# osudrl/cassie-mujoco-sim

Hardware: AMD Instinct MI355X
Metric: env-steps/sec (whole node) at N envs; max |qpos_err| vs CPU ref (higher is better)
Workload: dtype f64

## Files before the change

### cassie-mujoco-sim_amd/csrc/env_step_wave1.inc

```
    if constexpr (NW == 2) {
        if (wid == 1) {
            for (int sub1 = sub_start;;) {
                const int pb = isbody ? b : 0;
                const double mass = P->body_mass[pb];
                double iner[3], imat[9];
                for (int i = 0; i < 3; ++i) iner[i] = P->body_inertia[pb][i];
                for (int i = 0; i < 9; ++i) imat[i] = m->body_imat[pb][i];
                CK_STAMP(35);
                wv::block_barrier();
                if (wv::opaque(S.cmd[0])) return -1;
                wv::set_priority<(FEAT & FEAT_HFIELD) != 0 ? CK_PRIO_W1_FJ_HFIELD : CK_PRIO_W1_FJ>();
                CK_STAMP(36);
                double ximat[9] = {1, 0, 0, 0, 1, 0, 0, 0, 1};
                if (isbody && b > 0) {
                    double xm[9];
                    for (int i = 0; i < 9; ++i) xm[i] = S.x.s.xmat[b][i];
                    for (int i = 0; i < 3; ++i)
                        for (int c = 0; c < 3; ++c) ximat[3 * i + c] = xm[3 * i] * imat[c] + xm[3 * i + 1] * imat[3 + c] + xm[3 * i + 2] * imat[6 + c];
                }
                double col[NVP], colh[NVP];
                mass_matrix_columns<NVP, TOPO, FEAT, NW>(io, S, m, env, ids, mass, iner, ximat, col, colh);
                wv::publish(&S.cmd[3], sub1 + 1);
                CK_STAMP(38);
                factor_pair_by_height<NVP, TOPO, 0>(m, P, h, S, col, colh, lane);
                constexpr bool park_colh = NVP > 32;
                if constexpr (park_colh) {
                    if (isdof) {
#pragma unroll
                        for (int i = 0; i < NVP; ++i) {
                            if (i >= TOPO::nv) continue;
                            if (i == k_) S.dinvH[k_] = colh[i];
                            else if (i > k_ && LP::col_has(i, k_)) S.LHp[LP::col_idx(i, k_)] = colh[i];
                        }
                    }
                    wv::sync();
                }
                wv::wait_for(&S.cmd[4], sub1 + 1);
                if (wv::opaque(S.cmd[0])) return -1;
                if (io.drive_mode) {
                    if (io.integrate) drive_level_io(io, S, m, env, lane, sub1 == nsub - 1);
                    wv::sync();
                }
                CK_STAMP(4);
                {
                    const int kd = isdof ? k_ : 0;
                    const double kdamp = P->dof_damping[kd], kstiff = PS->dof_stiffness[kd], kref = PS->dof_springref[kd];
                    const double kgear = m->dof_gear[kd], klo = m->dof_ctrl_lo[kd], khi = m->dof_ctrl_hi[kd];
                    const int kq = m->dof_qadr[kd], ka = m->dof_act[kd];
                    wv::wait_for(&S.cmd[1], sub1 + 1);
                    bias_forces_and_qfrc_smooth<NVP, (NVP > 32)>(io, S, m, env, ids, kdamp, kstiff, kref, kgear, klo, khi, kq, ka);
                }
                const bool lastsub1 = sub1 == nsub - 1 || !io.integrate;
                const bool need_imu1 = lastsub1 || io.all_outputs_every_substep || (io.drive_mode && sub1 + 2 == nsub);
                const bool issens1 = lane < m->nsensor && (lastsub1 || io.drive_mode || io.all_outputs_every_substep);
                const int ls1 = issens1 ? lane : 0;
                const SensorConsts sens_c1 = request_sensor_consts(m, ls1);
                const int aslot1 = sensors_before_solve(io, S, m, env, issens1, ls1, sens_c1, need_imu1, lastsub1);
                CK_STAMP(47);
                wv::block_barrier();
                wv::set_priority<CK_PRIO_W1_JP>();
                CK_STAMP(39);
                if constexpr (WIDE) {
                    int it1 = 0, ng1 = 0;
                    const double f1 = wide_solve<NVP, TOPO>(S, m, P, 1, wv::opaque(S.x.turn[0]), sub1, it1, ng1);
                    (&S.c_solimp[0][0])[NROW + lane] = f1;
                }
                if constexpr (park_colh) {
#pragma unroll
                    for (int i = 0; i < NVP; ++i) {
                        double v = 0.0;
                        if (i < TOPO::nv && isdof) {
                            if (i == k_) v = S.dinvH[k_];
                            else if (i > k_ && LP::col_has(i, k_)) v = S.LHp[LP::col_idx(i, k_)];
                        }
                        colh[i] = v;
                    }
                    wv::sync();
                }
                factor_pair_by_height<NVP, TOPO, 1>(m, P, h, S, col, colh, lane);
                {
                    const bool lastsub = lastsub1, need_imu = need_imu1;
                    const int sb = sens_c1.sb, aslot = aslot1;
                    const int pf_u = lane < nu ? lane : 0, pf_ej = lane < njnt ? lane : 0;
                    const double pf_agear = m->act_gear[pf_u], pf_kdamp = P->dof_damping[isdof ? k_ : 0];
                    const int pf_adof = m->act_dofid[pf_u], pf_ejt = m->jnt_type[pf_ej], pf_eqa = m->jnt_qposadr[pf_ej], pf_eda = m->jnt_dofadr[pf_ej];
                    const double *const fbuf = &S.c_solimp[0][0];
                    double lrow[NVP];
                    constexpr bool stage_h_early = NVP <= 32;
                    if constexpr (stage_h_early) stage_factor_row<NVP, TOPO>(S, k_, isdof, lrow);
                    double lcol[NVP], lrowh[NVP];
                    if constexpr (stage_h_early) stage_factor_h<NVP, TOPO, 0>(S, k_, isdof, nv, lcol, lrowh);
                    const double rsdk = isdof ? S.rsd[k_] : 0.0;
                    const int kk = isdof ? k_ : 0;
                    constexpr bool stage_y = MAXR <= 31;
                    double ycolk[stage_y ? MAXR + 1 : 1];
                    if constexpr (stage_y) {
                        wv::wait_for(&S.cmd[2], sub1 + 1);
#pragma unroll
                        for (int r = 0; r <= MAXR; ++r) ycolk[r] = S.x.Yr[r][kk];
                    }
                    wv::block_barrier();
                    wv::set_priority<CK_PRIO_W1_PE>();
                    const double f = fbuf[lane], f_hi = WIDE ? fbuf[NROW + lane] : 0.0;
                    constexpr int FB = WIDE ? 2 * NROW : NROW;
                    const int ncon = (int)fbuf[FB], nefc = (int)fbuf[FB + 1], iters = (int)fbuf[FB + 2], nguarded = (int)fbuf[FB + 3];
                    double z, z1 = 0, z2 = 0, z3 = 0;
                    if constexpr (stage_y) {
                        z = isdof ? ycolk[MAXR] : 0.0;
#pragma unroll
                        for (int r = 0; r < MAXR; r += 4) {
                            if (r + 4 <= nefc) {
                                z += ycolk[r] * wv::readlane(f, r); z1 += ycolk[r + 1 < MAXR ? r + 1 : r] * wv::readlane(f, r + 1);
                                z2 += ycolk[r + 2 < MAXR ? r + 2 : r] * wv::readlane(f, r + 2); z3 += ycolk[r + 3 < MAXR ? r + 3 : r] * wv::readlane(f, r + 3);
                            } else {
#pragma unroll
                                for (int j = 0; j < 4; ++j) if (r + j < nefc && r + j < MAXR) z += ycolk[r + j < MAXR ? r + j : r] * wv::readlane(f, r + j);
                            }
                        }
                    } else {
                        z = isdof ? S.x.Yr[MAXR][k_] : 0.0;
                        auto frow = [&](int r) { if constexpr (WIDE) return r < NROW ? wv::readlane(f, r) : wv::readlane(f_hi, r - NROW); else return wv::readlane(f, r); };
                        int r = 0;
                        for (; r + 4 <= nefc; r += 4) {
                            const double y0 = S.x.Yr[r][kk], y1 = S.x.Yr[r + 1][kk], y2 = S.x.Yr[r + 2][kk], y3 = S.x.Yr[r + 3][kk];
                            z += y0 * frow(r); z1 += y1 * frow(r + 1);
                            z2 += y2 * frow(r + 2); z3 += y3 * frow(r + 3);
                        }
                        for (; r < nefc; ++r) z += S.x.Yr[r][kk] * frow(r);
                    }
                    z = (z + z1) + (z2 + z3);
                    if (!isdof) z = 0.0;
                    if (isdof) z *= rsdk;
                    if constexpr (stage_h_early) stage_factor_h<NVP, TOPO, 1>(S, k_, isdof, nv, lcol, lrowh);
                    const double dih = isdof ? S.dinvH[k_] : 0.0;
                    if constexpr (!stage_h_early) stage_factor_row<NVP, TOPO>(S, k_, isdof, lrow);
                    wv::sched_fence();
                    const double qacc = solve_forward<NVP, TOPO>(z, lrow, lane, nv);
                    {
                        const bool badv = isdof && (!(qacc == qacc) || fabs(qacc) > 1e10);
                        if (wv::ballot(badv) != 0ull) {
                            if (lane == 0) S.cmd[0] = 2;
                            wv::block_barrier();
                            return -1;
                        }
                    }
                    if (isdof) S.qacc[k_] = qacc;
                    const double av = pf_agear * S.qvel[pf_adof];
                    wv::sync();
                    CK_STAMP(12);
                    if (io.integrate) {
                        if constexpr (!stage_h_early) stage_factor_h<NVP, TOPO>(S, k_, isdof, nv, lcol, lrowh);
                        euler_step<NVP, TOPO>(S, m, lane, isdof, k_, nv, njnt, h, qacc, lcol, lrowh, dih, pf_kdamp, pf_ejt, pf_eqa, pf_eda);
                    }
                    CK_STAMP(13);
                    wv::block_barrier();
                    wv::set_priority<CK_PRIO_W1_EF>();
                    outputs_after_qacc(io, S, m, env, lane, isdof, k_, nu, qacc, aslot, sb, need_imu, lastsub, av, ncon, nefc, iters, nguarded);
                    CK_STAMP(14);
                }
                if (!io.integrate || ++sub1 >= nsub) return -1;
            }
        }
    }
```

### cassie-mujoco-sim_amd/csrc/physics_kernel.h

```cpp
#ifndef CASSIE_PHYSICS_KERNEL_H
#define CASSIE_PHYSICS_KERNEL_H

#include <wave.h>

#include "cm_model.h"
#include "topo_static.h"

#include "pk_types.h"
#include "pk_math.h"
#include "pk_safety.h"
#include "pk_collision.h"
#include "pk_factor_solve.h"
#include "pk_stages.h"
#include "pk_wide_solve.h"

namespace ck {


constexpr int ENV_STEP_WENT_DOWN = 1 << 20;

template <int NVP, class TOPO, int FEAT, int MAXR, int NW>
WV_DEVICE int env_step(const PhysIO &io, EnvShared<NVP, LPack<TOPO, NVP>::count, MAXR> &S, int env, int sub_start, int nsub) {
    typedef LPack<TOPO, NVP> LP;
    static_assert(NW == 1 || NW == 2, "one or two wavefronts per env");
    static_assert(NW == 1 || TOPO::is_static, "the two-wave form exists for the compile-time topologies");
    const int wid = NW == 2 ? wv::wave_id() : 0;
    if constexpr (NW == 2) { if (wid == 0) wv::set_priority<CK_PRIO_W0>(); }
    constexpr int prio_kin = (FEAT & FEAT_HFIELD) != 0 ? CK_PRIO_W0 : CK_PRIO_W0_KIN;

    static_assert(LP::covers() && LP::distinct(), "packed factor rows must hold every ancestor pair, each in its own slot");
    typedef EnvShared<NVP, LPack<TOPO, NVP>::count, MAXR> SH_T;
    constexpr int MAXC = SH_T::MAXC;
    constexpr bool WIDE = SH_T::WIDE;
    static_assert(!WIDE || (NW == 2 && MAXR == WIDE_ROWS), "the 127-row instantiation spreads its solve over the two wavefronts of an env");
    const ModelPtr m_launch = (ModelPtr)(io.models + (size_t)env * io.model_stride);
    ModelPtr m = m_launch;
    const ParamPtr P = io.envparams ? (ParamPtr)(io.envparams + (size_t)env) : (ParamPtr)&m_launch->params;
    const ParamPtr PG = m_launch->env_geom ? P : (ParamPtr)&m_launch->params, PS = m_launch->env_springs ? P : (ParamPtr)&m_launch->params;
    int lane = wv::lane();
    const int nq = m->nq, nv = m->nv, nu = m->nu, nbody = m->nbody, njnt = m->njnt;
    const int capr = m->maxefc < MAXR ? m->maxefc : MAXR, capc = m->maxcon < MAXC ? m->maxcon : MAXC;
    const bool can_hand_over = MAXR < WIDE_ROWS && io.has_next != 0 && io.progress != nullptr && (MAXR < m->maxefc || MAXC < m->maxcon);
    const double h = m->timestep;
    int warn = 0;

    if (NW == 1 || wid == 0) {
    if (lane == 0) { S.cmd[0] = 0; S.cmd[1] = 0; S.cmd[2] = 0; S.cmd[3] = 0; S.cmd[4] = 0; }
    if constexpr (WIDE) { if (lane == 0) { S.x.turn[0] = 0; S.x.turn[1] = 0; S.x.turn[2] = 0; S.x.turn[3] = 0; } }
    if (lane < nq) S.qpos[lane] = io.qpos[(size_t)env * io.sq + lane];
    if (lane < nv) {
        S.qvel[lane] = io.qvel[(size_t)env * io.sqv + lane];
        S.qacc_ws[lane] = io.qacc_warmstart[(size_t)env * io.sv + lane];
    }
    if (lane < nu) S.ctrl[lane] = io.ctrl[(size_t)env * io.su + lane];
    if (lane < NB && !wv::test_skip_com_init()) { S.com[lane][0] = 0.0; S.com[lane][1] = 0.0; S.com[lane][2] = 0.0; }
    if (io.drive_mode) {
        if (lane < m->nsensordata) S.sens[lane] = io.sensordata[(size_t)env * io.ssd + lane];
        if (lane < nu) S.actvel[lane] = io.actuator_velocity[(size_t)env * io.su + lane];
        drive_state_load(io, S, env, lane);
        drive_consts_load(io, S, m, env, lane);
    }
    }
    double time = io.time[env];

    int b = lane;
    bool isbody = b < nbody;
    const int depth = isbody ? m->body_depth[b] : -1;
    const int bparent = isbody ? m->body_parentid[b] : 0;
    const int broot = isbody ? m->body_rootid[b] : -1;
    const int bjn = isbody ? m->body_jntnum[b] : 0;
    const int bj0 = (isbody && bjn > 0) ? m->body_jntadr[b] : 0;
    const int bend = isbody ? m->body_subtreeend[b] : 0;
    const unsigned long long bdofmask = isbody ? m->body_dofmask[b] : 0ull;
    const int bjt = (isbody && bjn > 0) ? m->jnt_type[bj0] : -1;
    const int bjq = (isbody && bjn > 0) ? m->jnt_qposadr[bj0] : 0;
    int k_ = lane;
    bool isdof = k_ < nv;
    const int kjnt = isdof ? m->dof_jntid[k_] : 0;
    const int kbody = isdof ? m->dof_bodyid[k_] : 0;
    const int kjt = isdof ? m->jnt_type[kjnt] : -1;
    const int kda = isdof ? m->jnt_dofadr[kjnt] : 0;
    const int kqa = isdof ? m->jnt_qposadr[kjnt] : 0;
    const int kroot = isdof ? m->body_rootid[kbody] : 0;
    const int kbend = isdof ? m->body_subtreeend[kbody] : 0;
    const unsigned long long kdesc = isdof ? m->dof_descmask[k_] : 0ull;
    const unsigned long long kvelmask = isdof ? m->dof_velmask[k_] : 0ull;
    int kact = -1;
    for (int u = 0; u < nu; ++u) if (isdof && m->act_dofid[u] == k_) kact = u;
    const LaneIds ids = {nbody, nv, broot, bend, kjnt, kbody, kjt, kda, kroot, kbend, kdesc};
    wv::sync();

#include "env_step_wave1.inc"

    const float *env_hfield = nullptr;
    if constexpr ((FEAT & FEAT_HFIELD) != 0) {
        bool clamped;
        env_hfield = terrain_grid(io.hfield, io.hfield_stride, io.hfield_index, io.hfield_nterrain, env, &clamped);
        if (clamped && lane == 0 && wid == 0) wv::atomic_or(io.warn + env, WARN_TERRAIN_INDEX);
    }

    bool bailed = false, bailed_down = false;
    int sub = sub_start;
    for (; sub < nsub; ++sub) {
        const bool lastsub = sub == nsub - 1 || !io.integrate;
        const bool need_quat = lastsub || io.ext != nullptr || io.all_outputs_every_substep || (io.drive_mode && sub + 2 == nsub);
        {
            bool badv = false;
            if (lane < nq) { double v = S.qpos[lane]; badv |= !(v == v) || fabs(v) > 1e10; }
            if (lane < nv) { double v = S.qvel[lane]; badv |= !(v == v) || fabs(v) > 1e10; }
            if (wv::ballot(badv) != 0ull) {
                warn |= WARN_DIVERGED;
                if constexpr (NW == 2) { if (lane == 0) S.cmd[0] = 1; wv::block_barrier(); }
                break;
            }
        }
        if (io.drive_mode) {
        } else if (io.pd_ptarget) {
            if (lane < nu) {
                const size_t o = (size_t)env * io.su + lane;
                const double ratio = m->act_gear[lane], tmax = m->act_ctrlrange[lane][1];
                const double q = S.qpos[m->act_qposadr[lane]], qd = S.qvel[m->act_dofid[lane]];
                const double tau = io.pd_kp[o] * (io.pd_ptarget[o] - q) - io.pd_kd[o] * qd;
                const double wmax = m->act_maxrpm[lane] * (2.0 * 3.14159265358979323846 / 60.0);
                const double tlim = clampd(2 * tmax * (1 - fabs(ratio * qd) / wmax), 0.0, tmax);
                S.ctrl[lane] = copysign(fmin(fabs(tau / ratio), tlim), tau);
            }
            wv::sync();
        }
        CK_STAMP(0);
        if constexpr (NW == 2 && prio_kin != CK_PRIO_W0) wv::set_priority<prio_kin>();

        double Rl[9] = {1, 0, 0, 0, 1, 0, 0, 0, 1}, pl[3] = {0, 0, 0}, qlq[4] = {1, 0, 0, 0};
        constexpr int kin_rounds = [] {
            if constexpr (TOPO::is_static) { int r = 0, n = 1; while (n < TOPO::body_levels) { n *= 3; ++r; } return r < 1 ? 1 : r; }
            else return 3;
        }();
        int kanc[2 * kin_rounds];
#pragma unroll
        for (int r = 0; r < 2 * kin_rounds; ++r) kanc[r] = isbody ? m->body_anc3[b][r] : 0;
        const bool isfree = bjt == CM_JNT_FREE;
        if constexpr (TOPO::is_static) {
            {
                const auto *kr = &m->body_kin[isbody ? b : 0];
                const int nsl = kr->nslide, j0 = kr->jnt0, jr = kr->rot_jnt, jt = kr->rot_type, qa = kr->rot_qadr;
                int sqa[CM_MAXSLIDE];
                double sref[CM_MAXSLIDE], sax[CM_MAXSLIDE][3], spo[CM_MAXSLIDE][3];
#pragma unroll
                for (int sl = 0; sl < CM_MAXSLIDE; ++sl) {
                    sqa[sl] = kr->slide_qadr[sl]; sref[sl] = kr->slide_ref[sl];
                    for (int i = 0; i < 3; ++i) { sax[sl][i] = kr->slide_axis_p[sl][i]; spo[sl][i] = kr->slide_pos_p[sl][i]; }
                }
                const double jref = kr->rot_ref;
                double jp[3], ja[3], jpp[3], xl[3], q0[4];
                for (int i = 0; i < 3; ++i) { jp[i] = kr->rot_pos[i]; ja[i] = kr->rot_axis[i]; jpp[i] = kr->rot_pos_p[i]; xl[i] = kr->rot_axis_p[i]; }
                for (int i = 0; i < 9; ++i) Rl[i] = kr->mat[i];
                for (int i = 0; i < 3; ++i) pl[i] = kr->pos[i];
                for (int i = 0; i < 4; ++i) q0[i] = kr->quat[i];
#pragma unroll
                for (int sl = 0; sl < CM_MAXSLIDE; ++sl) {
                    const double d = S.qpos[sqa[sl]] - sref[sl];
                    if (sl < nsl) for (int i = 0; i < 3; ++i) { S.x.s.xanchor[j0 + sl][i] = pl[i] + spo[sl][i]; S.x.s.xaxis[j0 + sl][i] = sax[sl][i]; }
                    for (int i = 0; i < 3; ++i) pl[i] += sax[sl][i] * d;
                }
                for (int i = 0; i < 4; ++i) qlq[i] = q0[i];
                double sn, cs;
                sincos_bounded(jt == CM_JNT_HINGE ? 0.5 * (S.qpos[qa] - jref) : 0.0, sn, cs);
                if (jr >= 0) {
                    double qj[4];
                    if (jt == CM_JNT_HINGE) {
                        qj[0] = cs; qj[1] = ja[0] * sn; qj[2] = ja[1] * sn; qj[3] = ja[2] * sn;
                    } else {
                        const int qo = jt == CM_JNT_FREE ? qa + 3 : qa;
                        for (int i = 0; i < 4; ++i) qj[i] = S.qpos[qo + i];
                        normalize4_fast(qj);
                        if (jt == CM_JNT_FREE) for (int i = 0; i < 3; ++i) pl[i] = S.qpos[qa + i];
                    }
                    double al[3], Rq[9], Rn[9], r[3];
                    for (int i = 0; i < 3; ++i) { al[i] = pl[i] + jpp[i]; S.x.s.xanchor[jr][i] = al[i]; S.x.s.xaxis[jr][i] = xl[i]; }
                    quat2mat(Rq, qj);
                    for (int i = 0; i < 3; ++i)
                        for (int c = 0; c < 3; ++c) Rn[3 * i + c] = Rl[3 * i] * Rq[c] + Rl[3 * i + 1] * Rq[3 + c] + Rl[3 * i + 2] * Rq[6 + c];
                    for (int i = 0; i < 9; ++i) Rl[i] = Rn[i];
                    if (need_quat) mulquat(qlq, q0, qj);
                    mulmatvec3(r, Rl, jp);
                    for (int i = 0; i < 3; ++i) pl[i] = al[i] - r[i];
                }
            }
        } else
        if (isbody && b > 0) {
            double bpos[3], bq[4];
            for (int i = 0; i < 3; ++i) bpos[i] = m->body_pos[b][i];
            for (int i = 0; i < 4; ++i) bq[i] = m->body_quat[b][i];
            if (isfree) {
                for (int i = 0; i < 3; ++i) pl[i] = S.qpos[bjq + i];
                for (int i = 0; i < 4; ++i) qlq[i] = S.qpos[bjq + 3 + i];
                normalize4(qlq);
                quat2mat(Rl, qlq);
                for (int i = 0; i < 3; ++i) { S.x.s.xanchor[bj0][i] = pl[i]; S.x.s.xaxis[bj0][i] = (i == 2) ? 1.0 : 0.0; }
            } else {
                for (int i = 0; i < 9; ++i) Rl[i] = m->body_mat[b][i];
                for (int i = 0; i < 3; ++i) pl[i] = bpos[i];
                for (int i = 0; i < 4; ++i) qlq[i] = bq[i];
                int jt_n = 0, qa_n = 0;
                double jp_n[3] = {0, 0, 0}, ja_n[3] = {0, 0, 0}, ref_n = 0;
                if (bjn > 0) {
                    jt_n = m->jnt_type[bj0]; qa_n = m->jnt_qposadr[bj0]; ref_n = m->jnt_ref[bj0];
                    for (int i = 0; i < 3; ++i) { jp_n[i] = m->jnt_pos[bj0][i]; ja_n[i] = m->jnt_axis[bj0][i]; }
                }
                for (int jj = 0; jj < bjn; ++jj) {
                    const int j = bj0 + jj, jt = jt_n, qa = qa_n;
                    const double jref = ref_n;
                    double jp[3] = {jp_n[0], jp_n[1], jp_n[2]}, ja[3] = {ja_n[0], ja_n[1], ja_n[2]};
                    if (jj + 1 < bjn) {
                        jt_n = m->jnt_type[j + 1]; qa_n = m->jnt_qposadr[j + 1]; ref_n = m->jnt_ref[j + 1];
                        for (int i = 0; i < 3; ++i) { jp_n[i] = m->jnt_pos[j + 1][i]; ja_n[i] = m->jnt_axis[j + 1][i]; }
                    }
                    double al[3], xl[3];
                    mulmatvec3(al, Rl, jp);
                    for (int i = 0; i < 3; ++i) al[i] += pl[i];
                    mulmatvec3(xl, Rl, ja);
                    for (int i = 0; i < 3; ++i) { S.x.s.xanchor[j][i] = al[i]; S.x.s.xaxis[j][i] = xl[i]; }
                    if (jt == CM_JNT_SLIDE) {
                        const double sl = S.qpos[qa] - jref;
                        for (int i = 0; i < 3; ++i) pl[i] += xl[i] * sl;
                    } else {
                        double qj[4];
                        if (jt == CM_JNT_BALL) { for (int i = 0; i < 4; ++i) qj[i] = S.qpos[qa + i]; normalize4(qj); }
                        else {
                            const double ang = S.qpos[qa] - jref;
                            const double sn = sin(0.5 * ang);
                            qj[0] = cos(0.5 * ang); qj[1] = ja[0] * sn; qj[2] = ja[1] * sn; qj[3] = ja[2] * sn;
                        }
                        double Rq[9], Rn[9], r[3];
                        quat2mat(Rq, qj);
                        for (int i = 0; i < 3; ++i)
                            for (int c = 0; c < 3; ++c) Rn[3 * i + c] = Rl[3 * i] * Rq[c] + Rl[3 * i + 1] * Rq[3 + c] + Rl[3 * i + 2] * Rq[6 + c];
                        for (int i = 0; i < 9; ++i) Rl[i] = Rn[i];
                        if (need_quat) mulquat(qlq, qlq, qj);
                        mulmatvec3(r, Rl, jp);
                        for (int i = 0; i < 3; ++i) pl[i] = al[i] - r[i];
                    }
                }
            }
        }
        CK_STAMP(16);
        const int pf_b = isbody ? b : 0, pf_g = lane < m->ngeom ? lane : -1, pf_gs = pf_g >= 0 ? pf_g : 0;
        const int pf_jpb = lane < njnt ? m->jnt_parentbody[lane] : -1, pf_gb = m->geom_bodyid[pf_gs];
        const double pf_mass = P->body_mass[pf_b];
        double pf_ipos[3], pf_imat[9], pf_iner[3], pf_gpos[3], pf_gmat[9];
        for (int i = 0; i < 3; ++i) { pf_ipos[i] = P->body_ipos[pf_b][i]; pf_iner[i] = P->body_inertia[pf_b][i]; pf_gpos[i] = PG->geom_pos[pf_gs][i]; }
        for (int i = 0; i < 9; ++i) { pf_imat[i] = m->body_imat[pf_b][i]; pf_gmat[i] = PG->geom_mat[pf_gs][i]; }
        double xm[9], xp[3], xq[4];
        for (int i = 0; i < 9; ++i) xm[i] = Rl[i];
        for (int i = 0; i < 3; ++i) xp[i] = pl[i];
        for (int i = 0; i < 4; ++i) xq[i] = qlq[i];
        {
// ... 306 lines not shown
```

### cassie-mujoco-sim_amd/csrc/pk_stages.h

```cpp
#ifndef CASSIE_PK_STAGES_H
#define CASSIE_PK_STAGES_H

namespace ck {

WV_DEVICE int drive_sensor_slot(int i) { return i < 5 ? i : i + 3; }
WV_DEVICE int joint_sensor_slot(int j) { return j < 3 ? j + 5 : j + 10; }

#define WV_DRIVE_FN WV_DEVICE
template <class SH>
WV_DEVICE void drive_state_load(const PhysIO &io, SH &S, int env, int lane) {
    const cm_drive_state_t *ds = io.drive_state + env;
    const double *meas = io.meas + (size_t)env * CM_MEAS_DIM;
    if (lane < CM_NUM_DRIVES) {
        for (int k = 0; k < CM_DRIVE_FILTER_NB; ++k) S.drv_x[lane][k] = ds->drive_x[lane][k];
        for (int k = 0; k < CM_TORQUE_DELAY_CYCLES; ++k) S.drv_delay[lane][k] = ds->torque_delay[lane][k];
        S.drv_pos[lane] = meas[CM_MEAS_DRIVE_POS + lane]; S.drv_vel[lane] = meas[CM_MEAS_DRIVE_VEL + lane];
        if (lane == 0) S.drv_msg[0] = ds->safety_msg;
    } else if (lane < CM_NUM_DRIVES + CM_NUM_JOINTS) {
        const int j = lane - CM_NUM_DRIVES;
        for (int k = 0; k < CM_JOINT_FILTER_NB; ++k) S.drv_jx[j][k] = ds->joint_x[j][k];
        for (int k = 0; k < CM_JOINT_FILTER_NA; ++k) S.drv_jy[j][k] = ds->joint_y[j][k];
    }
}
template <class SH>
WV_DEVICE void drive_state_store(const PhysIO &io, SH &S, int env, int lane) {
    cm_drive_state_t *ds = io.drive_state + env;
    if (lane < CM_NUM_DRIVES) {
        for (int k = 0; k < CM_DRIVE_FILTER_NB; ++k) ds->drive_x[lane][k] = S.drv_x[lane][k];
        for (int k = 0; k < CM_TORQUE_DELAY_CYCLES; ++k) ds->torque_delay[lane][k] = S.drv_delay[lane][k];
        if (lane == 0) ds->safety_msg = S.drv_msg[0];
    } else if (lane < CM_NUM_DRIVES + CM_NUM_JOINTS) {
        const int j = lane - CM_NUM_DRIVES;
        for (int k = 0; k < CM_JOINT_FILTER_NB; ++k) ds->joint_x[j][k] = S.drv_jx[j][k];
        for (int k = 0; k < CM_JOINT_FILTER_NA; ++k) ds->joint_y[j][k] = S.drv_jy[j][k];
    }
}

enum { DRVC_RATIO = 0, DRVC_TMAX, DRVC_WMAX, DRVC_COUNTS, DRVC_SCALE, DRVC_U_OR_PT, DRVC_STO_OR_DT, DRVC_FF, DRVC_KP, DRVC_KD };
template <class SH>
WV_DEVICE void drive_consts_load(const PhysIO &io, SH &S, ModelPtr m, int env, int lane) {
    const double TWO_PI = 2 * 3.14159265358979323846, PI = 3.14159265358979323846;
    const int nu = m->nu;
    if (lane < CM_NUM_DRIVES) {
        const int i = lane, bits = m->sensor_bits[drive_sensor_slot(i)];
        const double ratio = m->act_gear[i], counts = (double)(1 << bits);
        double *c = S.drv_c[i];
        c[DRVC_RATIO] = ratio; c[DRVC_TMAX] = m->act_ctrlrange[i][1];
        c[DRVC_WMAX] = wv::div_rn(wv::mul_rn(wv::mul_rn(m->act_maxrpm[i], 2.0), PI), 60.0);
        c[DRVC_COUNTS] = counts; c[DRVC_SCALE] = wv::div_rn(wv::div_rn(TWO_PI, counts), ratio);
        if (io.drive_mode == CM_DRIVE_TORQUE) {
            c[DRVC_U_OR_PT] = io.drive_cmd[(size_t)env * (nu + 1) + i];
            c[DRVC_STO_OR_DT] = io.drive_cmd[(size_t)env * (nu + 1) + nu] != 0.0 ? 1.0 : 0.0;
            c[DRVC_FF] = 0.0; c[DRVC_KP] = 0.0; c[DRVC_KD] = 0.0;
        } else {
            const size_t o = (size_t)env * nu + i;
            c[DRVC_U_OR_PT] = io.pd_ptarget[o]; c[DRVC_STO_OR_DT] = io.pd_dtarget ? io.pd_dtarget[o] : 0.0;
            c[DRVC_FF] = io.pd_torque ? io.pd_torque[o] : 0.0; c[DRVC_KP] = io.pd_kp[o]; c[DRVC_KD] = io.pd_kd[o];
            if (i == 0) S.drv_msg[1] = (io.drive_mode == CM_DRIVE_PD_SAFE && io.drive_cmd && io.drive_cmd[(size_t)env * (nu + 1) + nu] != 0.0) ? 1 : 0;
        }
    } else if (lane < CM_NUM_DRIVES + CM_NUM_JOINTS) {
        const int j = lane - CM_NUM_DRIVES, bits = m->sensor_bits[joint_sensor_slot(j)];
        const double counts = (double)(1 << bits);
        S.drv_jc[j][0] = counts; S.drv_jc[j][1] = wv::div_rn(TWO_PI, counts);
    }
}

template <class SH>
WV_DRIVE_FN void drive_level_io(const PhysIO &io, SH &S, ModelPtr m, int env, int lane, bool write_meas) {
    const double TWO_PI = 2 * 3.14159265358979323846, PI = 3.14159265358979323846;
    double *meas = io.meas + (size_t)env * CM_MEAS_DIM;
    double u_safe = 0.0;
    if (io.drive_mode == CM_DRIVE_PD_SAFE) {
        int msg = 0;
        const bool sto = S.drv_msg[1] != 0;
        if (lane < CM_NUM_DRIVES) {
            double qq[CM_NUM_DRIVES];
            for (int k = 0; k < CM_NUM_DRIVES; ++k) qq[k] = S.drv_pos[k];
            const double *c = S.drv_c[lane];
            const double wk = S.drv_vel[lane];
            const double uk = wv::add_rn(wv::add_rn(c[DRVC_FF], wv::mul_rn(c[DRVC_KP], wv::sub_rn(c[DRVC_U_OR_PT], S.drv_pos[lane]))), wv::mul_rn(c[DRVC_KD], wv::sub_rn(c[DRVC_STO_OR_DT], wk)));
            u_safe = safety::drive_torque(lane, uk, qq, wk, safety::torque_limit(lane), sto, &msg);
        }
        const bool lim = wv::ballot((msg & safety::MSG_LIMIT) != 0) != 0ull, trq = wv::ballot((msg & safety::MSG_TORQUE) != 0) != 0ull;
        wv::sync();
        if (lane == 0 && io.integrate) S.drv_msg[0] |= (lim ? safety::MSG_LIMIT : 0) | (trq ? safety::MSG_TORQUE : 0);
    }
    if (lane < CM_NUM_DRIVES) {
        const int i = lane;
        double cst[10];
        for (int k = 0; k < 10; ++k) cst[k] = S.drv_c[i][k];
        const double ratio = cst[DRVC_RATIO], tmax = cst[DRVC_TMAX], wmax = cst[DRVC_WMAX];
        double u;
        bool sto = false;
        if (io.drive_mode == CM_DRIVE_TORQUE) {
            u = cst[DRVC_U_OR_PT];
            sto = cst[DRVC_STO_OR_DT] != 0.0;
        } else if (io.drive_mode == CM_DRIVE_PD_SAFE) {
            u = u_safe;
            sto = S.drv_msg[1] != 0;
        } else {
            const double p = S.drv_pos[i], v = S.drv_vel[i];
            const double pt = cst[DRVC_U_OR_PT], dt = cst[DRVC_STO_OR_DT], ff = cst[DRVC_FF];
            u = wv::add_rn(wv::add_rn(ff, wv::mul_rn(cst[DRVC_KP], wv::sub_rn(pt, p))), wv::mul_rn(cst[DRVC_KD], wv::sub_rn(dt, v)));
        }
        const double w = S.actvel[i];
        double tlim = wv::mul_rn(wv::mul_rn(2.0, tmax), wv::sub_rn(1.0, wv::div_rn(fabs(w), wmax)));
        tlim = fmax(fmin(tlim, tmax), 0.0);
        if (sto) u = 0.0;
        const double tau = copysign(fmin(fabs(wv::div_rn(u, ratio)), tlim), u);
        double dl[CM_TORQUE_DELAY_CYCLES];
        for (int k = 0; k < CM_TORQUE_DELAY_CYCLES; ++k) dl[k] = S.drv_delay[i][k];
        const double ctrl_i = dl[CM_TORQUE_DELAY_CYCLES - 1];
        for (int k = CM_TORQUE_DELAY_CYCLES - 1; k > 0; --k) S.drv_delay[i][k] = dl[k - 1];
        S.drv_delay[i][0] = tau;
        S.ctrl[i] = ctrl_i;
        const int slot = drive_sensor_slot(i);
        const double counts = cst[DRVC_COUNTS], scale = cst[DRVC_SCALE];
        const int ev = (int)wv::mul_rn(wv::div_rn(S.sens[slot], TWO_PI), counts);
        const double pos = wv::mul_rn((double)ev, scale);
        int x[CM_DRIVE_FILTER_NB];
        bool allzero = true;
        for (int k = 0; k < CM_DRIVE_FILTER_NB; ++k) { x[k] = S.drv_x[i][k]; allzero &= x[k] == 0; }
        if (allzero) for (int k = 0; k < CM_DRIVE_FILTER_NB; ++k) x[k] = ev;
        for (int k = CM_DRIVE_FILTER_NB - 1; k > 0; --k) x[k] = x[k - 1];
        x[0] = ev;
        const int fir[CM_DRIVE_FILTER_NB] = {2727, 534, -2658, -795, 72, 110, 19, -6, -3};
        int y = 0;
        for (int k = 0; k < CM_DRIVE_FILTER_NB; ++k) { y += x[k] * fir[k]; S.drv_x[i][k] = x[k]; }
        const double vel = wv::div_rn(wv::mul_rn((double)y, scale), PI);
        S.drv_pos[i] = pos; S.drv_vel[i] = vel;
        if (write_meas) {
            meas[CM_MEAS_DRIVE_POS + i] = pos; meas[CM_MEAS_DRIVE_VEL + i] = vel;
            meas[CM_MEAS_DRIVE_TORQUE + i] = wv::mul_rn(ctrl_i, ratio);
        }
    } else if (lane < CM_NUM_DRIVES + CM_NUM_JOINTS) {
        const int j = lane - CM_NUM_DRIVES, slot = joint_sensor_slot(j);
        const double counts = S.drv_jc[j][0], scale = S.drv_jc[j][1];
        const int ev = (int)wv::mul_rn(wv::div_rn(S.sens[slot], TWO_PI), counts);
        const double pos = wv::mul_rn((double)ev, scale);
        double x[CM_JOINT_FILTER_NB], yv[CM_JOINT_FILTER_NA];
        bool allzero = true;
        for (int k = 0; k < CM_JOINT_FILTER_NB; ++k) { x[k] = S.drv_jx[j][k]; allzero &= x[k] == 0; }
        for (int k = 0; k < CM_JOINT_FILTER_NA; ++k) yv[k] = S.drv_jy[j][k];
        if (allzero) for (int k = 0; k < CM_JOINT_FILTER_NB; ++k) x[k] = pos;
        for (int k = CM_JOINT_FILTER_NB - 1; k > 0; --k) x[k] = x[k - 1];
        x[0] = pos;
        for (int k = CM_JOINT_FILTER_NA - 1; k > 0; --k) yv[k] = yv[k - 1];
        const double fb[CM_JOINT_FILTER_NB] = {12.348, 12.348, -12.348, -12.348}, fa[CM_JOINT_FILTER_NA] = {1.0, -1.7658, 0.79045};
        double y0 = 0.0;
        for (int k = 0; k < CM_JOINT_FILTER_NB; ++k) y0 = wv::add_rn(y0, wv::mul_rn(x[k], fb[k]));
        for (int k = 1; k < CM_JOINT_FILTER_NA; ++k) y0 = wv::sub_rn(y0, wv::mul_rn(yv[k], fa[k]));
        yv[0] = y0;
        for (int k = 0; k < CM_JOINT_FILTER_NB; ++k) S.drv_jx[j][k] = x[k];
        for (int k = 0; k < CM_JOINT_FILTER_NA; ++k) S.drv_jy[j][k] = yv[k];
        if (write_meas) { meas[CM_MEAS_JOINT_POS + j] = pos; meas[CM_MEAS_JOINT_VEL + j] = y0; }
    } else if (lane < 29) {
        if (write_meas) meas[CM_MEAS_ORIENTATION + (lane - 16)] = S.sens[lane];
    }
}

enum { FEAT_HFIELD = 1, FEAT_WAVEPAIRS = 2, FEAT_ALL = 3 };

struct LaneIds { int nbody, nv, broot, bend, kjnt, kbody, kjt, kda, kroot, kbend; unsigned long long kdesc; };

template <int NVP, class TOPO, int FEAT, int NW, class SH>
WV_DEVICE void mass_matrix_columns(const PhysIO &io, SH &S, ModelPtr m, int env, const LaneIds &ids, const double pf_mass, const double (&pf_iner)[3],
                                   const double (&ximat)[9], double (&col)[NVP], double (&colh)[NVP]) {
    const int nbody = ids.nbody, nv = ids.nv, broot = ids.broot, bend = ids.bend, kjnt = ids.kjnt, kbody = ids.kbody, kjt = ids.kjt, kda = ids.kda, kroot = ids.kroot;
    const unsigned long long kdesc = ids.kdesc;
    int lane = wv::fresh_lane(), b = lane, k_ = lane;
    bool isbody = b < nbody, isdof = k_ < nv;
    constexpr bool cbuf_over_anchors = NW == 2 && (FEAT & FEAT_HFIELD) != 0;
    static_assert(!cbuf_over_anchors || NVP <= CM_MAXJNT, "crb . cdof (NVP x 6) must fit the xanchor + xaxis tiles");
    static_assert(offsetof(decltype(S.x.s), xaxis) - offsetof(decltype(S.x.s), xanchor) == sizeof(double) * CM_MAXJNT * 3, "xanchor and xaxis are contiguous");
    double (*const cbuf)[6] = cbuf_over_anchors ? reinterpret_cast<double (*)[6]>(&S.x.s.xanchor[0][0]) : S.x.s.buf;
    const double bmass = (isbody && b > 0) ? pf_mass : 0.0;
    {
        const double px = isbody ? S.x.s.xipos[b < NB ? b : 0][0] : 0.0, py = isbody ? S.x.s.xipos[b < NB ? b : 0][1] : 0.0,
                     pz = isbody ? S.x.s.xipos[b < NB ? b : 0][2] : 0.0;
        for (int ri = 0; ri < m->nroot; ++ri) {
            const int r = m->root_body[ri], e = m->body_subtreeend[r];
            const double w = (isbody && b >= r && b < e) ? bmass : 0.0;
            const double sm = wv::wave_sum(w), sx = wv::wave_sum(w * px), sy = wv::wave_sum(w * py), sz = wv::wave_sum(w * pz);
            if (lane == 0) {
                if (sm < CM_MINVAL) { S.com[r][0] = S.x.s.xipos[r][0]; S.com[r][1] = S.x.s.xipos[r][1]; S.com[r][2] = S.x.s.xipos[r][2]; }
                else { const double inv = 1.0 / sm; S.com[r][0] = sx * inv; S.com[r][1] = sy * inv; S.com[r][2] = sz * inv; }
            }
        }
    }
    wv::sync();
    CK_STAMP(18);
    if (lane < NB) {
        double ci[10] = {0, 0, 0, 0, 0, 0, 0, 0, 0, 0};
        if (isbody && b > 0) {
            const double I0 = pf_iner[0], I1 = pf_iner[1], I2 = pf_iner[2];
            const double *c = S.com[broot];
            double dif[3] = {S.x.s.xipos[b][0] - c[0], S.x.s.xipos[b][1] - c[1], S.x.s.xipos[b][2] - c[2]};
            double d2 = dot3(dif, dif);
            const double *R = ximat;
            double W00 = R[0] * I0 * R[0] + R[1] * I1 * R[1] + R[2] * I2 * R[2];
            double W11 = R[3] * I0 * R[3] + R[4] * I1 * R[4] + R[5] * I2 * R[5];
            double W22 = R[6] * I0 * R[6] + R[7] * I1 * R[7] + R[8] * I2 * R[8];
            double W01 = R[0] * I0 * R[3] + R[1] * I1 * R[4] + R[2] * I2 * R[5];
            double W02 = R[0] * I0 * R[6] + R[1] * I1 * R[7] + R[2] * I2 * R[8];
            double W12 = R[3] * I0 * R[6] + R[4] * I1 * R[7] + R[5] * I2 * R[8];
            ci[0] = W00 + bmass * (d2 - dif[0] * dif[0]);
            ci[1] = W11 + bmass * (d2 - dif[1] * dif[1]);
            ci[2] = W22 + bmass * (d2 - dif[2] * dif[2]);
            ci[3] = W01 - bmass * dif[0] * dif[1];
            ci[4] = W02 - bmass * dif[0] * dif[2];
            ci[5] = W12 - bmass * dif[1] * dif[2];
            ci[6] = bmass * dif[0]; ci[7] = bmass * dif[1]; ci[8] = bmass * dif[2]; ci[9] = bmass;
        }
        for (int i = 0; i < 10; ++i) S.x.s.cinert[lane][i] = ci[i];
    }
    {
    double cd[6] = {0, 0, 0, 0, 0, 0};
    if (isdof) {
        const double *c = S.com[kroot];
        double off[3] = {c[0] - S.x.s.xanchor[kjnt][0], c[1] - S.x.s.xanchor[kjnt][1], c[2] - S.x.s.xanchor[kjnt][2]};
        const int sub_k = k_ - kda;
        if (kjt == CM_JNT_SLIDE) {
            for (int i = 0; i < 3; ++i) cd[3 + i] = S.x.s.xaxis[kjnt][i];
        } else if (kjt == CM_JNT_HINGE) {
            for (int i = 0; i < 3; ++i) cd[i] = S.x.s.xaxis[kjnt][i];
            cross3(cd + 3, cd, off);
        } else if (kjt == CM_JNT_FREE && sub_k < 3) {
            cd[3 + sub_k] = 1.0;
        } else {
            const int a = (kjt == CM_JNT_FREE) ? sub_k - 3 : sub_k;
            cd[0] = S.x.s.xmat[kbody][a]; cd[1] = S.x.s.xmat[kbody][3 + a]; cd[2] = S.x.s.xmat[kbody][6 + a];
            cross3(cd + 3, cd, off);
        }
    }
    if (lane < NVP) for (int i = 0; i < 6; ++i) S.cdof[lane][i] = cd[i];
    }
    wv::sync();
    CK_STAMP(2);

    {
        const int mi = lane & 15, mk = lane >> 4;
        const unsigned mine = (isbody && b > 0) ? (unsigned)(((1ull << bend) - 1ull) ^ ((1ull << b) - 1ull)) : 0u;
        const unsigned w0 = (unsigned)wv::shfl_i((int)mine, mi) >> mk, w1 = (unsigned)wv::shfl_i((int)mine, 16 + mi) >> mk;
        double bv[NB / 4];
#pragma unroll
        for (int kb = 0; kb < NB / 4; ++kb) { const double v = S.x.s.cinert[4 * kb + mk][mi < 10 ? mi : 0]; bv[kb] = mi < 10 ? v : 0.0; }
        wv::mfma_acc d0a = {{0, 0, 0, 0}}, d0b = {{0, 0, 0, 0}}, d1a = {{0, 0, 0, 0}}, d1b = {{0, 0, 0, 0}};
#pragma unroll
        for (int kb = 0; kb < NB / 4; kb += 2)
            wv::mfma_f64_16x16x4_x4((double)((w0 >> (4 * kb)) & 1u), bv[kb], d0a, (double)((w1 >> (4 * kb)) & 1u), bv[kb], d1a,
                                    (double)((w0 >> (4 * kb + 4)) & 1u), bv[kb + 1], d0b, (double)((w1 >> (4 * kb + 4)) & 1u), bv[kb + 1], d1b);
        wv::mfma_f64_drain4(d0a, d0b, d1a, d1b);
        if (mi < 10) {
#pragma unroll
            for (int v = 0; v < 4; ++v) {
                S.x.s.crb[mk + 4 * v][mi] = d0a.c[v] + d0b.c[v];
                S.x.s.crb[16 + mk + 4 * v][mi] = d1a.c[v] + d1b.c[v];
            }
        }
    }
    wv::sync();
    CK_STAMP(19);
    if (lane < NVP) {
        double bf[6] = {0, 0, 0, 0, 0, 0}, cd[6];
        for (int i = 0; i < 6; ++i) cd[i] = S.cdof[lane][i];
        if (isdof) mul_inert_vec(bf, S.x.s.crb[kbody], cd);
        for (int i = 0; i < 6; ++i) cbuf[lane][i] = bf[i];
    }
    wv::sync();
    CK_STAMP(20);
    double cdm[6];
    if constexpr (NVP == 32) {
        const int hk = lane & 31, roff = lane < 32 ? 0 : 16;
        const unsigned hdesc = (unsigned)wv::shfl_i((int)(unsigned)kdesc, hk) >> roff;
        for (int i = 0; i < 6; ++i) cdm[i] = S.cdof[hk][i];
        const double (*bufr)[6] = &cbuf[roff];
        double part[16];
#pragma unroll
        for (int i0 = 0; i0 < 16; i0 += 8) {
            double bb[8][6];
#pragma unroll
            for (int ii = 0; ii < 8; ++ii)
#pragma unroll
                for (int t = 0; t < 6; ++t) bb[ii][t] = bufr[i0 + ii][t];
            wv::sched_fence();
#pragma unroll
            for (int ii = 0; ii < 8; ++ii) {
                const double v = (cdm[0] * bb[ii][0] + cdm[1] * bb[ii][1]) + (cdm[2] * bb[ii][2] + cdm[3] * bb[ii][3]) + (cdm[4] * bb[ii][4] + cdm[5] * bb[ii][5]);
                part[i0 + ii] = ((hdesc >> (i0 + ii)) & 1u) ? v : 0.0;
            }
        }
#pragma unroll
        for (int i = 0; i < 16; ++i) {
            const double up = wv::from_upper_half(part[i]);
            col[i] = part[i]; colh[i] = part[i];
            col[16 + i] = up; colh[16 + i] = up;
        }
    } else {
    for (int i = 0; i < 6; ++i) cdm[i] = S.cdof[lane < NVP ? lane : 0][i];
#pragma unroll
    for (int i0 = 0; i0 < NVP; i0 += 8) {
        double bb[8][6];
#pragma unroll
        for (int ii = 0; ii < 8; ++ii)
#pragma unroll
            for (int t = 0; t < 6; ++t) bb[ii][t] = cbuf[i0 + ii][t];
        wv::sched_fence();
#pragma unroll
        for (int ii = 0; ii < 8; ++ii) {
            const int i = i0 + ii;
            double v = (cdm[0] * bb[ii][0] + cdm[1] * bb[ii][1]) + (cdm[2] * bb[ii][2] + cdm[3] * bb[ii][3]) + (cdm[4] * bb[ii][4] + cdm[5] * bb[ii][5]);
// ... 271 lines not shown
```

Baseline: 27.61 million.

## Compute drive-level controller ahead of mass-matrix work in wave 1

```diff
diff --git a/cassie-mujoco-sim_amd/csrc/env_step_wave1.inc b/cassie-mujoco-sim_amd/csrc/env_step_wave1.inc
--- a/cassie-mujoco-sim_amd/csrc/env_step_wave1.inc
+++ b/cassie-mujoco-sim_amd/csrc/env_step_wave1.inc
@@ -1,6 +1,15 @@
     if constexpr (NW == 2) {
         if (wid == 1) {
+            constexpr bool drive_ahead = drive_ahead_of_f<NVP>;
             for (int sub1 = sub_start;;) {
+#ifdef CK_PROF_SUBSTEP
+                io.prof = sub1 == nsub - 1 - (CK_PROF_SUBSTEP) ? io_launch.prof : nullptr;
+#endif
+                DriveResult drv = {0.0, 0.0, 0.0, 0, false, false};
+                if constexpr (drive_ahead) {
+                    if constexpr ((FEAT & FEAT_HFIELD) == 0) CK_STAMP(44);
+                    if (io.drive_mode && io.integrate) { wv::sync(); drv = drive_level_compute(io, S, lane); }
+                }
                 const int pb = isbody ? b : 0;
                 const double mass = P->body_mass[pb];
                 double iner[3], imat[9];
@@ -37,8 +46,12 @@
                 }
                 wv::wait_for(&S.cmd[4], sub1 + 1);
                 if (wv::opaque(S.cmd[0])) return -1;
+                CK_STAMP(15);
                 if (io.drive_mode) {
-                    if (io.integrate) drive_level_io(io, S, m, env, lane, sub1 == nsub - 1);
+                    if (io.integrate) {
+                        if constexpr (drive_ahead) drive_level_commit(io, S, env, lane, drv, sub1 == nsub - 1);
+                        else drive_level_io(io, S, m, env, lane, sub1 == nsub - 1);
+                    }
                     wv::sync();
                 }
                 CK_STAMP(4);
diff --git a/cassie-mujoco-sim_amd/csrc/physics_kernel.h b/cassie-mujoco-sim_amd/csrc/physics_kernel.h
--- a/cassie-mujoco-sim_amd/csrc/physics_kernel.h
+++ b/cassie-mujoco-sim_amd/csrc/physics_kernel.h
@@ -20,7 +20,12 @@
 constexpr int ENV_STEP_WENT_DOWN = 1 << 20;
 
 template <int NVP, class TOPO, int FEAT, int MAXR, int NW>
-WV_DEVICE int env_step(const PhysIO &io, EnvShared<NVP, LPack<TOPO, NVP>::count, MAXR> &S, int env, int sub_start, int nsub) {
+WV_DEVICE int env_step(const PhysIO &io_launch, EnvShared<NVP, LPack<TOPO, NVP>::count, MAXR> &S, int env, int sub_start, int nsub) {
+#ifdef CK_PROF_SUBSTEP
+    PhysIO io = io_launch;
+#else
+    const PhysIO &io = io_launch;
+#endif
     typedef LPack<TOPO, NVP> LP;
     static_assert(NW == 1 || NW == 2, "one or two wavefronts per env");
     static_assert(NW == 1 || TOPO::is_static, "the two-wave form exists for the compile-time topologies");
@@ -89,6 +94,7 @@
     for (int u = 0; u < nu; ++u) if (isdof && m->act_dofid[u] == k_) kact = u;
     const LaneIds ids = {nbody, nv, broot, bend, kjnt, kbody, kjt, kda, kroot, kbend, kdesc};
     wv::sync();
+    if constexpr (NW == 2 && drive_ahead_of_f<NVP>) { if (io.drive_mode && io.integrate) wv::block_barrier(); }
 
 #include "env_step_wave1.inc"
 
@@ -102,6 +108,9 @@
     bool bailed = false, bailed_down = false;
     int sub = sub_start;
     for (; sub < nsub; ++sub) {
+#ifdef CK_PROF_SUBSTEP
+        io.prof = sub == nsub - 1 - (CK_PROF_SUBSTEP) ? io_launch.prof : nullptr;
+#endif
         const bool lastsub = sub == nsub - 1 || !io.integrate;
         const bool need_quat = lastsub || io.ext != nullptr || io.all_outputs_every_substep || (io.drive_mode && sub + 2 == nsub);
         {
diff --git a/cassie-mujoco-sim_amd/csrc/pk_stages.h b/cassie-mujoco-sim_amd/csrc/pk_stages.h
--- a/cassie-mujoco-sim_amd/csrc/pk_stages.h
+++ b/cassie-mujoco-sim_amd/csrc/pk_stages.h
@@ -65,10 +65,29 @@
     }
 }
 
-template <class SH>
-WV_DRIVE_FN void drive_level_io(const PhysIO &io, SH &S, ModelPtr m, int env, int lane, bool write_meas) {
+#ifndef CK_W1_DRIVE_AHEAD
+#define CK_W1_DRIVE_AHEAD 1
+#endif
+template <int NVP> constexpr bool drive_ahead_of_f = CK_W1_DRIVE_AHEAD != 0 && NVP <= 32;
+
+template <class T, int N> WV_DRIVE_FN void history_shift(T (&x)[N]) { for (int k = N - 1; k > 0; --k) x[k] = x[k - 1]; }
+template <class T, int N> WV_DRIVE_FN void history_push(T (&x)[N], const T v) {
+    bool allzero = true;
+    for (int k = 0; k < N; ++k) allzero &= x[k] == 0;
+    if (allzero) for (int k = 0; k < N; ++k) x[k] = v;
+    history_shift(x);
+    x[0] = v;
+}
+struct DriveResult {
+    double a;
+    double pos, vel;
+    int ev;
+    bool lim, trq;
+};
+template <class SH>
+WV_DRIVE_FN DriveResult drive_level_compute(const PhysIO &io, const SH &S, int lane) {
     const double TWO_PI = 2 * 3.14159265358979323846, PI = 3.14159265358979323846;
-    double *meas = io.meas + (size_t)env * CM_MEAS_DIM;
+    DriveResult res = {0.0, 0.0, 0.0, 0, false, false};
     double u_safe = 0.0;
     if (io.drive_mode == CM_DRIVE_PD_SAFE) {
         int msg = 0;
@@ -81,9 +100,7 @@
             const double uk = wv::add_rn(wv::add_rn(c[DRVC_FF], wv::mul_rn(c[DRVC_KP], wv::sub_rn(c[DRVC_U_OR_PT], S.drv_pos[lane]))), wv::mul_rn(c[DRVC_KD], wv::sub_rn(c[DRVC_STO_OR_DT], wk)));
             u_safe = safety::drive_torque(lane, uk, qq, wk, safety::torque_limit(lane), sto, &msg);
         }
-        const bool lim = wv::ballot((msg & safety::MSG_LIMIT) != 0) != 0ull, trq = wv::ballot((msg & safety::MSG_TORQUE) != 0) != 0ull;
-        wv::sync();
-        if (lane == 0 && io.integrate) S.drv_msg[0] |= (lim ? safety::MSG_LIMIT : 0) | (trq ? safety::MSG_TORQUE : 0);
+        res.lim = wv::ballot((msg & safety::MSG_LIMIT) != 0) != 0ull; res.trq = wv::ballot((msg & safety::MSG_TORQUE) != 0) != 0ull;
     }
     if (lane < CM_NUM_DRIVES) {
         const int i = lane;
@@ -107,56 +124,81 @@
         double tlim = wv::mul_rn(wv::mul_rn(2.0, tmax), wv::sub_rn(1.0, wv::div_rn(fabs(w), wmax)));
         tlim = fmax(fmin(tlim, tmax), 0.0);
         if (sto) u = 0.0;
-        const double tau = copysign(fmin(fabs(wv::div_rn(u, ratio)), tlim), u);
-        double dl[CM_TORQUE_DELAY_CYCLES];
-        for (int k = 0; k < CM_TORQUE_DELAY_CYCLES; ++k) dl[k] = S.drv_delay[i][k];
-        const double ctrl_i = dl[CM_TORQUE_DELAY_CYCLES - 1];
-        for (int k = CM_TORQUE_DELAY_CYCLES - 1; k > 0; --k) S.drv_delay[i][k] = dl[k - 1];
-        S.drv_delay[i][0] = tau;
-        S.ctrl[i] = ctrl_i;
+        res.a = copysign(fmin(fabs(wv::div_rn(u, ratio)), tlim), u);
         const int slot = drive_sensor_slot(i);
         const double counts = cst[DRVC_COUNTS], scale = cst[DRVC_SCALE];
         const int ev = (int)wv::mul_rn(wv::div_rn(S.sens[slot], TWO_PI), counts);
-        const double pos = wv::mul_rn((double)ev, scale);
+        res.ev = ev;
+        res.pos = wv::mul_rn((double)ev, scale);
         int x[CM_DRIVE_FILTER_NB];
-        bool allzero = true;
-        for (int k = 0; k < CM_DRIVE_FILTER_NB; ++k) { x[k] = S.drv_x[i][k]; allzero &= x[k] == 0; }
-        if (allzero) for (int k = 0; k < CM_DRIVE_FILTER_NB; ++k) x[k] = ev;
-        for (int k = CM_DRIVE_FILTER_NB - 1; k > 0; --k) x[k] = x[k - 1];
-        x[0] = ev;
+        for (int k = 0; k < CM_DRIVE_FILTER_NB; ++k) x[k] = S.drv_x[i][k];
+        history_push(x, ev);
         const int fir[CM_DRIVE_FILTER_NB] = {2727, 534, -2658, -795, 72, 110, 19, -6, -3};
         int y = 0;
-        for (int k = 0; k < CM_DRIVE_FILTER_NB; ++k) { y += x[k] * fir[k]; S.drv_x[i][k] = x[k]; }
-        const double vel = wv::div_rn(wv::mul_rn((double)y, scale), PI);
-        S.drv_pos[i] = pos; S.drv_vel[i] = vel;
-        if (write_meas) {
-            meas[CM_MEAS_DRIVE_POS + i] = pos; meas[CM_MEAS_DRIVE_VEL + i] = vel;
-            meas[CM_MEAS_DRIVE_TORQUE + i] = wv::mul_rn(ctrl_i, ratio);
-        }
+        for (int k = 0; k < CM_DRIVE_FILTER_NB; ++k) y += x[k] * fir[k];
+        res.vel = wv::div_rn(wv::mul_rn((double)y, scale), PI);
     } else if (lane < CM_NUM_DRIVES + CM_NUM_JOINTS) {
         const int j = lane - CM_NUM_DRIVES, slot = joint_sensor_slot(j);
         const double counts = S.drv_jc[j][0], scale = S.drv_jc[j][1];
         const int ev = (int)wv::mul_rn(wv::div_rn(S.sens[slot], TWO_PI), counts);
         const double pos = wv::mul_rn((double)ev, scale);
+        res.pos = pos;
         double x[CM_JOINT_FILTER_NB], yv[CM_JOINT_FILTER_NA];
-        bool allzero = true;
-        for (int k = 0; k < CM_JOINT_FILTER_NB; ++k) { x[k] = S.drv_jx[j][k]; allzero &= x[k] == 0; }
+        for (int k = 0; k < CM_JOINT_FILTER_NB; ++k) x[k] = S.drv_jx[j][k];
         for (int k = 0; k < CM_JOINT_FILTER_NA; ++k) yv[k] = S.drv_jy[j][k];
-        if (allzero) for (int k = 0; k < CM_JOINT_FILTER_NB; ++k) x[k] = pos;
-        for (int k = CM_JOINT_FILTER_NB - 1; k > 0; --k) x[k] = x[k - 1];
-        x[0] = pos;
-        for (int k = CM_JOINT_FILTER_NA - 1; k > 0; --k) yv[k] = yv[k - 1];
+        history_push(x, pos);
+        history_shift(yv);
         const double fb[CM_JOINT_FILTER_NB] = {12.348, 12.348, -12.348, -12.348}, fa[CM_JOINT_FILTER_NA] = {1.0, -1.7658, 0.79045};
         double y0 = 0.0;
         for (int k = 0; k < CM_JOINT_FILTER_NB; ++k) y0 = wv::add_rn(y0, wv::mul_rn(x[k], fb[k]));
         for (int k = 1; k < CM_JOINT_FILTER_NA; ++k) y0 = wv::sub_rn(y0, wv::mul_rn(yv[k], fa[k]));
-        yv[0] = y0;
+        res.a = y0;
+    }
+    return res;
+}
+template <class SH>
+WV_DRIVE_FN void drive_level_commit(const PhysIO &io, SH &S, int env, int lane, const DriveResult &res, bool write_meas) {
+    double *meas = io.meas + (size_t)env * CM_MEAS_DIM;
+    wv::sync();
+    if (io.drive_mode == CM_DRIVE_PD_SAFE && lane == 0 && io.integrate) S.drv_msg[0] |= (res.lim ? safety::MSG_LIMIT : 0) | (res.trq ? safety::MSG_TORQUE : 0);
+    if (lane < CM_NUM_DRIVES) {
+        const int i = lane, ev = res.ev;
+        double dl[CM_TORQUE_DELAY_CYCLES];
+        for (int k = 0; k < CM_TORQUE_DELAY_CYCLES; ++k) dl[k] = S.drv_delay[i][k];
+        const double ctrl_i = dl[CM_TORQUE_DELAY_CYCLES - 1];
+        for (int k = CM_TORQUE_DELAY_CYCLES - 1; k > 0; --k) S.drv_delay[i][k] = dl[k - 1];
+        S.drv_delay[i][0] = res.a;
+        S.ctrl[i] = ctrl_i;
+        int x[CM_DRIVE_FILTER_NB];
+        for (int k = 0; k < CM_DRIVE_FILTER_NB; ++k) x[k] = S.drv_x[i][k];
+        history_push(x, ev);
+        for (int k = 0; k < CM_DRIVE_FILTER_NB; ++k) S.drv_x[i][k] = x[k];
+        S.drv_pos[i] = res.pos; S.drv_vel[i] = res.vel;
+        if (write_meas) {
+            meas[CM_MEAS_DRIVE_POS + i] = res.pos; meas[CM_MEAS_DRIVE_VEL + i] = res.vel;
+            meas[CM_MEAS_DRIVE_TORQUE + i] = wv::mul_rn(ctrl_i, S.drv_c[i][DRVC_RATIO]);
+        }
+    } else if (lane < CM_NUM_DRIVES + CM_NUM_JOINTS) {
+        const int j = lane - CM_NUM_DRIVES;
+        const double pos = res.pos;
+        double x[CM_JOINT_FILTER_NB], yv[CM_JOINT_FILTER_NA];
+        for (int k = 0; k < CM_JOINT_FILTER_NB; ++k) x[k] = S.drv_jx[j][k];
+        for (int k = 0; k < CM_JOINT_FILTER_NA; ++k) yv[k] = S.drv_jy[j][k];
+        history_push(x, pos);
+        history_shift(yv);
+        yv[0] = res.a;
         for (int k = 0; k < CM_JOINT_FILTER_NB; ++k) S.drv_jx[j][k] = x[k];
         for (int k = 0; k < CM_JOINT_FILTER_NA; ++k) S.drv_jy[j][k] = yv[k];
-        if (write_meas) { meas[CM_MEAS_JOINT_POS + j] = pos; meas[CM_MEAS_JOINT_VEL + j] = y0; }
+        if (write_meas) { meas[CM_MEAS_JOINT_POS + j] = pos; meas[CM_MEAS_JOINT_VEL + j] = res.a; }
     } else if (lane < 29) {
         if (write_meas) meas[CM_MEAS_ORIENTATION + (lane - 16)] = S.sens[lane];
     }
+}
+template <class SH>
+WV_DRIVE_FN void drive_level_io(const PhysIO &io, SH &S, ModelPtr m, int env, int lane, bool write_meas) {
+    (void)m;
+    const DriveResult res = drive_level_compute(io, S, lane);
+    drive_level_commit(io, S, env, lane, res, write_meas);
 }
 
 enum { FEAT_HFIELD = 1, FEAT_WAVEPAIRS = 2, FEAT_ALL = 3 };
```

Result: no change. 27.84 million, median of 6 (+0.8%).
